# wilsonCernWq/qaray

Hardware: AMD Instinct MI355X
Metric: Msamples/s (1 sample = 1 camera path), Cornell box 1080p@512spp (higher is better)
Workload: dtype f32

## Files before the change

### qaray_amd/csrc/hip/qa_capi.hip

```cpp
#include <hip/hip_runtime.h>

#include <algorithm>
#include <cstddef>
#include <cstring>
#include <new>

#include "qa_ctx.h"

static int EnsurePlanSlab(qa_ctx *c)
{
  const size_t threads = (size_t) c->numCUs * 8 * QA_BLOCK;
  const bool area = c->plan.area, many = !area && c->plan.shadowLights.size() > QA_CS_LIGHT_BATCH;
  float **slab = area ? &c->dAreaSlab : many ? &c->dSurfSlab : nullptr;
  if (slab && !*slab) {
    void *p = nullptr;
    HIP_TRY(hipMalloc(&p, threads * (area ? kAreaLogFloats : 13) * sizeof(float)));
    c->sceneAllocs.push_back(p);
    c->statSceneAllocs++;
    *slab = static_cast<float *>(p);
  }
  c->ds.areaScratch = area ? c->dAreaSlab : nullptr;
  c->ds.csSurf = many ? c->dSurfSlab : nullptr;
  return QA_OK;
}
// ... 351 lines not shown
  if (nbytes) *nbytes = c->hostBlob.size();
  if (!out || capacity < c->hostBlob.size()) return Fail(QA_EINVAL, "output smaller than the scene blob");
  if (int rc = FetchDeviceTexels(c)) return rc;
  memcpy(out, c->hostBlob.data(), c->hostBlob.size());
  return QA_OK;
}

int qa_get_scene_stats(qa_ctx *c, uint64_t out[4])
{
  if (!c || !out) return Fail(QA_EINVAL, "null argument");
  out[0] = c->statMeshBuilds; out[1] = c->statSceneAllocs; out[2] = c->statBytesCopied; out[3] = c->statEdits;
  return QA_OK;
}

int qa_synchronize(qa_ctx *c)
{
  if (int rc = Enter(c)) return rc;
  HIP_TRY(hipStreamSynchronize(c->stream));
  return DrainEvents(c);
}

static int SetStop(qa_ctx *c, int stop)
{
  if (!c) return Fail(QA_EINVAL, "null context");
  __atomic_store_n(c->hStop, stop, __ATOMIC_SEQ_CST);
  return QA_OK;
}
int qa_request_stop(qa_ctx *c) { return SetStop(c, 1); }
int qa_clear_stop(qa_ctx *c) { return SetStop(c, 0); }

int qa_get_counters(qa_ctx *c, qa_counters *out)
{
  if (!c || !out) return Fail(QA_EINVAL, "null argument");
  if (int rc = qa_synchronize(c)) return rc;
  DCounters h;
  HIP_TRY(hipMemcpy(&h, c->dCounters, sizeof(h), hipMemcpyDeviceToHost));
  out->samples = h.samples;
  out->casts_normal = h.casts_normal;
  out->casts_shadow = h.casts_shadow;
  out->bvh_nodes = h.bvh_nodes;
  out->tri_tests = h.tri_tests;
  out->pixels = h.pixels;
#ifdef QA_STAMPS
  {
    const double w = (double) std::max<unsigned long long>(h.stamp[9], 1), k = (double) std::max<unsigned long long>(h.stamp[0], 1);
    fprintf(stderr, "[stamps] waves %llu, iterations/wave %.0f, cycles/wave %.3e | share of wave time: fetch+start %.3f, closest %.3f (mesh walks %.3f), shade %.3f, "
            "direct light %.3f (shadow mesh walks %.3f), sample end %.3f, miss branch %.3f, hit before shading %.3f, spawn %.3f\n", h.stamp[9], h.stamp[8] / w, k / w, h.stamp[1] / k, h.stamp[2] / k, h.stamp[3] / k,
            h.stamp[4] / k, h.stamp[5] / k, h.stamp[6] / k, h.stamp[7] / k, h.stamp[10] / k, h.stamp[11] / k, h.stamp[12] / k);
    if (h.stamp[19] || h.stamp[21])
      fprintf(stderr, "[stamps] waves without a camera ray: mesh walks of their closest-hit sweeps %.3f (the camera rays': %.3f), after the sweep %.3f | last-cast queries %.3f (mesh walks %.3f), %llu lanes asked again (of %llu casts)\n",
              h.stamp[19] / k, (h.stamp[3] - (double) h.stamp[19]) / k, h.stamp[20] / k, h.stamp[21] / k, h.stamp[22] / k, h.stamp[23], (unsigned long long) h.casts_normal);
    if (!c->integ[kCs].fn && h.stamp[16])
      fprintf(stderr, "[stamps] turns of empty tiles: %llu of %llu turns (%.3f), share of wave time %.4f\n", h.stamp[16], h.stamp[8], (double) h.stamp[16] / (double) std::max<unsigned long long>(h.stamp[8], 1), h.stamp[15] / k);
    if (c->integ[kCs].fn && h.stamp[11])
      fprintf(stderr, "[stamps] cooperative walks: %llu rounds, %.1f of 64 lanes hold an item on average (lane occupancy of the walks %.3f); %.3f of the rounds are leaf rounds; 'mesh walks' above = the rounds alone\n", h.stamp[11],
              (double) h.stamp[10] / (double) h.stamp[11], (double) h.stamp[10] / (64.0 * (double) h.stamp[11]), (double) h.stamp[12] / (double) h.stamp[11]);
    if (c->integ[kCs].fn)
      fprintf(stderr, "[stamps] closest-hit sweeps without their rounds %.3f, winners' details %.3f, shadow sweeps without their rounds %.3f; lanes sent to the exact walks: %llu closest, %llu shadow (of %llu + %llu casts)\n",
              (h.stamp[13] - (double) h.stamp[3]) / k, h.stamp[14] / k, (h.stamp[17] - (double) h.stamp[6]) / k, h.stamp[15], h.stamp[16], (unsigned long long) h.casts_normal, (unsigned long long) h.casts_shadow);
  }
#endif
  return QA_OK;
}
int qa_reset_counters(qa_ctx *c)
{
  if (!c) return Fail(QA_EINVAL, "null context");
  if (int rc = qa_synchronize(c)) return rc;
  HIP_TRY(hipMemset(c->dCounters, 0, sizeof(DCounters)));
  if (c->wf.dStats) HIP_TRY(hipMemset(c->wf.dStats, 0, sizeof(WfStats)));
  c->wf.iterations = c->wf.raysClosest = c->wf.raysShadow = c->wf.jobs = c->wf.redo = 0;
  return QA_OK;
}

int qa_get_staged_stats(qa_ctx *c, uint64_t out[QA_STAGED_STATS])
{
  if (!c || !out) return Fail(QA_EINVAL, "null argument");
  if (int rc = qa_synchronize(c)) return rc;
  WfStats st;
  memset(&st, 0, sizeof(st));
  if (c->wf.dStats) HIP_TRY(hipMemcpy(&st, c->wf.dStats, sizeof(st), hipMemcpyDeviceToHost));
  const uint64_t v[QA_STAGED_STATS] = {c->wf.iterations, c->wf.raysClosest, c->wf.raysShadow, c->wf.jobs, c->wf.redo, st.jobs, st.nodeSteps,
                                       st.leafSteps, st.triTests, st.redo, st.suspended, st.laneSlots, st.waveRounds};
  memcpy(out, v, sizeof(v));
  return QA_OK;
}

int qa_set_pipeline(qa_ctx *c, int mode)
{
  if (!c) return Fail(QA_EINVAL, "null context");
  if (mode < QA_PIPE_MEGA || mode > QA_PIPE_AUTO) return Fail(QA_EINVAL, "pipeline mode must be QA_PIPE_MEGA, QA_PIPE_STAGED or QA_PIPE_AUTO");
  c->wf.mode = mode;
  c->wf.modeSet = true;
  if (c->haveScene) SetKernelName(c);
  return QA_OK;
}

const char *qa_get_kernel_name(qa_ctx *c)
{
  if (!c || !c->haveScene) return "";
  return c->launchedName.empty() ? c->kernelName.c_str() : c->launchedName.c_str();
}

int qa_get_kernel_time(qa_ctx *c, double *total_ms, uint64_t *launches)
{
  if (!c || !total_ms || !launches) return Fail(QA_EINVAL, "null argument");
  HIP_TRY(hipSetDevice(c->device));
// ... 54 lines not shown
```

### qaray_amd/csrc/hip/qa_kernel.h

```cpp
#pragma once
#include <hip/hip_runtime.h>

#include <type_traits>

#include "qa_device_math.h"
#include "qa_scene_dev.h"
#include "qa_seed.h"
#include "qa_texture_dev.h"
#include "qa_tilecull.h"
#include "qa_emptytile.h"

namespace qa {

#ifndef QA_MIN_WAVES
#define QA_MIN_WAVES 4
#endif
#define QA_BIAS 0.005f
#define QA_DX 0.01f
#ifdef QA_WAVE_TALLIES
#define QA_TALLY(x) (x) += (unsigned long long) __popcll(__ballot(1))
#else
#define QA_LANE_TALLIES 1
#define QA_TALLY(x) (x)++
#endif
// ... 712 lines not shown
    any |= hit;
  }
  if (any) {
    for (int a = h.node; a >= 0; a = instAt<RES>(sc, a).parent) {
      if (a == 0 && sc.rootIdentity) {
        h.N = normalize(h.N);
        break;
      }
      const qa_instance &in = instAt<RES>(sc, a);
      h.p = mulMV(in.tm, h.p) + ld3(in.pos);
      h.N = normalize(mulTMV(in.itm, h.N));
    }
  }
  return any;
}

template <bool RES, bool STATS>
__device__ __forceinline__ float shadow(const SceneMem<RES> mem, const DScene &sc, const Ray &world, float t_max,
                                        uint32_t *stack, DCounters &cnt)
{
  QA_TALLY(cnt.casts_shadow);
  Hit h;
  h.z = t_max;
  h.node = -1;
  const Ray r0 = rootRay<RES>(sc, world);
  GroupRay grp;
  grp.node = -1;
  grp.ray = r0;
  for (int k = 1; k < sc.num_inst; ++k) {
    const int type = instAt<RES>(sc, k).obj_type;
    if (type == QA_OBJ_NONE) continue;
    const Ray r = localRayInGroup<RES>(sc, k, r0, grp);
    bool hit;
    if (type == QA_OBJ_SPHERE) hit = hitSphere(r, h, k, false);
    else if (type == QA_OBJ_PLANE) hit = hitPlane(r, h, k, false);
    else {
      TriPick pick;
      QA_T(tm0)
      hit = hitMesh<RES, STATS>(mem, meshAt<RES>(sc, instAt<RES>(sc, k).mesh), r, h, k, false, stack, cnt, pick, sc.stackDepth);
      QA_TACC(cnt.sl[6], tm0)
    }
    if (hit) return 0.0f;
  }
  return 1.0f;
}

#ifndef QA_LEAF_SWEEP
#define QA_LEAF_SWEEP 1
#endif
#ifndef QA_LEAF_SWEEP_SORTED
#define QA_LEAF_SWEEP_SORTED 1
#endif

typedef const __attribute__((address_space(4))) uint32_t *QaLeafPtr;
__device__ __forceinline__ uint32_t sweepLeafBoxes(QaLeafPtr rec, uint32_t j0, uint32_t j1, const Ray &ray, f3 pLo, f3 pHi, f3 drcp, bool fastSlab, float limit)
{
  uint32_t mask = 0;
#pragma unroll 4
  for (uint32_t j = j0; j < j1; ++j) {
    QaLeafPtr r = rec + 8 * (size_t) j;
    const f3 bmin = F3(asF(r[0]), asF(r[1]), asF(r[2])), bmax = F3(asF(r[3]), asF(r[4]), asF(r[5]));
    float entry, exit_;
    if (fastSlab) {
#if QA_FMA_SLAB
      boxEntryExitPadFma(pLo, pHi, drcp, bmin, bmax, entry, exit_);
#else
      boxEntryExitPadFast(pLo, pHi, drcp, bmin, bmax, entry, exit_);
#endif
    } else boxEntryExitPad(pLo, pHi, ray.d, drcp, bmin, bmax, entry, exit_);
    mask |= (entry <= limit && entry <= exit_) ? (1u << (j - j0)) : 0u;
  }
  return mask;
}

__device__ __forceinline__ bool sweepLeaves(const uint4 *table, uint32_t numLeaves, const uint4 *ftris, const Ray &ray, f3 drcp, bool fastSlab,
                                            float &hz, uint32_t &best, bool &tie, float pad)
{
  f3 pLo = ray.p + F3(pad, pad, pad), pHi = ray.p - F3(pad, pad, pad);
  if (QA_FMA_SLAB && fastSlab) { pLo = slabRayTerm(pLo, drcp); pHi = slabRayTerm(pHi, drcp); }
  QaLeafPtr rec = (QaLeafPtr) table;
  const uint32_t n0 = numLeaves < 32u ? numLeaves : 32u;
  uint32_t lo = sweepLeafBoxes(rec, 0, n0, ray, pLo, pHi, drcp, fastSlab, hz), hi = 0;
  if (numLeaves > 32u) hi = sweepLeafBoxes(rec, 32, numLeaves, ray, pLo, pHi, drcp, fastSlab, hz);
  typedef const __attribute__((address_space(1))) uint32_t *WordPtr;
  WordPtr words = (WordPtr) table;
  while (lo | hi) {
    uint32_t j;
    if (lo) { j = (uint32_t) __ffs((int) lo) - 1u; lo &= lo - 1u; }
    else { j = 31u + (uint32_t) __ffs((int) hi); hi &= hi - 1u; }
    const uint32_t word = words[8 * (size_t) j + 6];
    const uint32_t count = ((word >> QA_BVH_COUNT_SHIFT) & QA_BVH_COUNT_MASK) + 1;
    const uint32_t first = word & QA_BVH_OFFSET_MASK;
    for (uint32_t i = 0; i < count; ++i) {
      const uint4 *t = ftris + 3 * (size_t) (first + i);
      const uint4 t2 = t[2];
      if (hitTriangleZTie<true>(t[0], t[1], t2, ray, hz, tie)) {
        best = t2.w >> 2;
        return true;
      }
    }
  }
  return false;
}

template <bool RES>
__device__ __forceinline__ bool blocksMesh(const SceneMem<RES> mem, const DMesh &m, const Ray &ray, float limit, uint32_t *stack,
                                           DCounters &cnt, bool &again, const uint4 *leafTable = nullptr)
{
  const f3 drcp = F3(1.f / ray.d.x, 1.f / ray.d.y, 1.f / ray.d.z);
  const bool fastSlab = !__any(qabs(ray.d.x) < 1e-7f || qabs(ray.d.y) < 1e-7f || qabs(ray.d.z) < 1e-7f);
  float meshExit;
  bool gate;
  {
    float entry;
    if (fastSlab) boxEntryExitFast(ray, drcp, ld3(m.bmin), ld3(m.bmax), entry, meshExit);
    else boxEntryExit(ray, drcp, ld3(m.bmin), ld3(m.bmax), entry, meshExit);
    if (entry > meshExit) return false;
    gate = !(entry > limit);
  }
  if (m.num_faces == 0) return false;
  if (!m.useFast) {
    again = true;
    return false;
  }
  const uint4 *nodes = mem.img + m.resNodes, *fnodes = mem.img + m.resFNodes, *ftris = mem.img + m.resFTris;
  const float oMax = qmax(qmax(qabs(ray.p.x), qabs(ray.p.y)), qabs(ray.p.z));
  const float pad = fastWalkPad(m.invH, m.absMax, oMax);
  float hz = limit;
  uint32_t bestF = 0;
  bool tie = false;
  bool hit;
#if QA_LEAF_SWEEP
  const uint32_t numLeaves = __builtin_amdgcn_readfirstlane(m.numLeaves);
  if (leafTable && numLeaves >= 2 && numLeaves <= QA_TILE_LEAF_CAP)
    hit = sweepLeaves(leafTable + __builtin_amdgcn_readfirstlane(m.resLeaves) + (QA_LEAF_SWEEP_SORTED ? 2 * (size_t) numLeaves : 0), numLeaves, ftris, ray,
                      drcp, fastSlab, hz, bestF, tie, pad);
  else
#endif
  hit = walkBVH<true, false, false, QA_BLOCK, QA_FMA_SLAB != 0>(fnodes, ftris, m.frootData, ray, drcp, fastSlab, hz, false, stack, cnt, bestF, tie, pad);
  if (tie) {
    again = true;
    return false;
  }
  if (!hit) {
    if (limit > meshExit) {
      const float theta = ((QA_SLACK_SCALE * 1.8e-5f) * m.invH) * (oMax + m.absMax) + QA_SLACK_SCALE * 2e-5f;
      const float lim = (theta * theta) * dot(ray.d, ray.d);
      bool parallel = m.numNormals == 0;
      const float4 *nrm = reinterpret_cast<const float4 *>(mem.img + m.resNormals);
      for (uint32_t i = 0; i < m.numNormals; ++i) {
        const float4 n = nrm[i];
        const float dn = __builtin_fmaf(ray.d.x, n.x, __builtin_fmaf(ray.d.y, n.y, ray.d.z * n.z));
        parallel = parallel || (dn * dn <= lim);
      }
      if (parallel) {
        uint32_t bestR = 0;
        hz = limit;
        return walkBVH<false, false>(nodes, mem.img + m.resTris, m.rootData, ray, drcp, fastSlab, hz, false, stack, cnt, bestR, tie);
      }
    }
    return false;
  }
  if (!gate || !refReaches(nodes, bestF >> 15, ray, drcp, fastSlab, limit)) {
    again = true;
    return false;
  }
  return true;
}

#ifndef QA_LAST_CAST_ANYHIT
#define QA_LAST_CAST_ANYHIT 1
#endif
template <bool RES>
__device__ __forceinline__ void closestEmitter(const SceneMem<RES> mem, const DScene &sc, const Ray &world, uint32_t *stack,
                                               DCounters &cnt, bool &drawn, int &emitSet)
{
  const Ray r0 = rootRay<RES>(sc, world);
  Hit h;
  h.z = QA_BIGFLOAT;
  h.node = -1;
  for (int k = 1; k < sc.num_inst; ++k) {
    const int type = instAt<RES>(sc, k).obj_type;
    if (type == QA_OBJ_NONE) continue;
    const Ray r = localRay<RES>(sc, k, r0);
    if (type == QA_OBJ_SPHERE) hitSphere(r, h, k, true);
    else if (type == QA_OBJ_PLANE) hitPlane(r, h, k, true);
    else {
      TriPick pick;
      hitMesh<RES, false, true, false>(mem, meshAt<RES>(sc, instAt<RES>(sc, k).mesh), r, h, k, true, stack, cnt, pick, sc.stackDepth);
    }
  }
  drawn = h.node >= 0;
  emitSet = -1;
  for (uint32_t rest = sc.lastCastGlow; rest; rest &= rest - 1) {
    const int k = __ffs((int) rest) - 1;
    if (k == h.node) emitSet = instAt<RES>(sc, k).mtlset;
  }
}

template <bool RES>
__device__ __forceinline__ bool lastCastQuery(const SceneMem<RES> mem, const DScene &sc, const Ray &world, uint32_t *stack,
                                              DCounters &cnt, bool &drawn, int &emitSet)
{
  const Ray r0 = rootRay<RES>(sc, world);
  const uint32_t glow = sc.lastCastGlow;
  Hit h;
  h.z = QA_BIGFLOAT;
  int G = -1, setG = -1;
  for (uint32_t rest = glow; rest; rest &= rest - 1) {
    const int k = __ffs((int) rest) - 1;
    if (k >= sc.num_inst) break;
    const qa_instance &in = instAt<RES>(sc, k);
    const Ray r = localRay<RES>(sc, k, r0);
    const bool hit = in.obj_type == QA_OBJ_SPHERE ? hitSphere(r, h, k, false) : hitPlane(r, h, k, false);
    if (hit) {
      G = k;
      setG = in.mtlset;
    }
  }
  const float tG = h.z;
  const float tGup = __uint_as_float(__float_as_uint(tG) + 1u);
  bool blocked = false, again = false;
  for (int k = 1; k < sc.num_inst; ++k) {
    if ((glow >> k) & 1u) continue;
    const int type = instAt<RES>(sc, k).obj_type;
    if (type == QA_OBJ_NONE) continue;
    const bool open = !blocked && !again;
    if (!__any(open)) break;
    if (open) {
      const float limit = G < 0 ? QA_BIGFLOAT : (k < G ? tGup : tG);
      const Ray r = localRay<RES>(sc, k, r0);
      Hit b;
      b.z = limit;
      if (type == QA_OBJ_SPHERE) blocked = hitSphere(r, b, k, false);
      else if (type == QA_OBJ_PLANE) blocked = hitPlane(r, b, k, false);
      else {
        QA_T(tm0)
        blocked = blocksMesh<RES>(mem, meshAt<RES>(sc, instAt<RES>(sc, k).mesh), r, limit, stack, cnt, again, sc.lastCast == 2u ? sc.resident : nullptr);
        QA_TACC(cnt.sl[22], tm0)
      }
    }
  }
  drawn = blocked || G >= 0;
  emitSet = blocked ? -1 : setG;
  return !again;
}

__device__ __forceinline__ float inverseSquareFalloff(f3 v) { return qmin(1.f, 1.f / dot(v, v)); }

__device__ __forceinline__ float spotAttenuation(const qa_light &l, f3 p)
{
  const f3 d = normalize(p - ld3(l.position));
  const float cosTheta = dot(d, ld3(l.direction));
  if (cosTheta < 0) return 0;
  const float rr = qsqrt(1.f - cosTheta * cosTheta) / cosTheta;
  if (rr > l.outer) return 0;
  return rr < l.inner ? 1.f : qpowf((l.outer - rr) / (l.outer - l.inner), 2.f);
}

template <bool RES, bool STATS>
__device__ __forceinline__ f3 illuminate(const SceneMem<RES> mem, const DScene &sc, const qa_light &l, f3 p,
                                         uint32_t *stack, DCounters &cnt, uint32_t &rng)
{
  const f3 intensity = ld3(l.intensity);
  if (l.type != QA_LIGHT_DIRECT && l.size > 0.01f) {
    int spp = 16, n = 0;
    float inshadow = 0.0f;
    while (n < spp) {
      const f3 dir = (ld3(l.position) + uniformBall(rng, l.size)) - p;
      Ray r;
      r.p = p;
      r.d = normalize(dir);
      inshadow += (shadow<RES, STATS>(mem, sc, r, length(dir), stack, cnt) - inshadow) * inverseSquareFalloff(dir) / (float) (n + 1);
      n++;
      if (inshadow > 0.f && inshadow < 1.f) spp = 64;
    }
    f3 I = intensity * inshadow;
    if (l.type == QA_LIGHT_SPOT) I = I * spotAttenuation(l, p);
    return I;
  }
  if (l.type == QA_LIGHT_DIRECT) {
    Ray r;
    r.p = p;
    r.d = normalize(-ld3(l.direction));
    return intensity * shadow<RES, STATS>(mem, sc, r, QA_BIGFLOAT, stack, cnt);
  }
  const f3 dir = ld3(l.position) - p;
  Ray r;
  r.p = p;
  r.d = normalize(dir);
  f3 I = (intensity * shadow<RES, STATS>(mem, sc, r, length(dir), stack, cnt)) * inverseSquareFalloff(dir);
// ... 429 lines not shown
```

### qaray_amd/csrc/hip/qa_kernel_lastcast_body.h

```cpp
  extern __shared__ uint4 s_dyn[];
  SceneMem<RES> mem;
  mem.img = s_dyn;
  static_assert(RES, "the last-cast query belongs to the resident variant without lights");
  for (uint32_t i = threadIdx.x; i < sc.residentVec4; i += QA_BLOCK) s_dyn[i] = sc.resident[i];
  __syncthreads();
  uint32_t *stack = reinterpret_cast<uint32_t *>(s_dyn + sc.residentVec4) + threadIdx.x;
  float *acc = reinterpret_cast<float *>(stack + (size_t) sc.stackDepth * QA_BLOCK - threadIdx.x) + threadIdx.x;
  const uint4 *mtlTable = s_dyn + sc.resMaterials;
  for (int i = 12; i < QA_LANE_SLOTS_RES; ++i) acc[i * QA_BLOCK] = 0.f;
  constexpr bool TL = true;
  uint32_t *tileList = nullptr;
  if (rp.tile_lists > 0 && !(sc.cam.dof > 0.1f))
    tileList = reinterpret_cast<uint32_t *>(s_dyn + sc.residentVec4) + ((size_t) sc.stackDepth + QA_LANE_SLOTS_RES) * QA_BLOCK +
               __builtin_amdgcn_readfirstlane(threadIdx.x / 64) * QA_TILE_LIST_DWORDS;

  const int rw = rp.x1 - rp.x0, rh = rp.y1 - rp.y0;
  const unsigned tilesX = (unsigned) (rw + 7) / 8;
  const unsigned numTiles = tilesX * (unsigned) rp.own_tile_rows;
  const unsigned total = numTiles * (rp.chunk_spp ? rp.num_chunks : 1u) * 64u;
  const unsigned lane = __lane_id();
  unsigned curTile = 0xFFFFFFFFu, curChunk = 0;
  int chunkEnd = 0x7FFFFFFF;

  DCounters cnt = {};
#ifdef QA_STAMPS
  __shared__ unsigned long long s_stamps[QA_BLOCK / 64][QA_NSTAMPS];
  cnt.sl = s_stamps[threadIdx.x / 64];
  if (__lane_id() < QA_NSTAMPS) cnt.sl[__lane_id()] = 0;
#endif
  QA_T(tKernel)
  TexTables tt;
  tt.blob = sc.blob;
  tt.texels = sc.texels;
  tt.texOff = sc.texOff;
  tt.texmap = sc.texmap;
  tt.tex = sc.tex;
  tt.filter = sc.texFilter;
  RayDiff pathDiff;
  pathDiff.dx = pathDiff.dy = F3(0, 0, 1);

  uint32_t rng = 1;
  bool alive = true, needPixel = true;
#if QA_EMPTY_TILES
#ifdef QA_WAVE_TALLIES
#define QA_TALLY_N(x, n) (x) += (unsigned long long) (n) * (unsigned long long) __popcll(__ballot(1))
#else
#define QA_TALLY_N(x, n) (x) += (unsigned long long) (n)
#endif
#ifdef QA_STAMPS
  bool tileEmpty = false;
#define QA_EMPTY_ASK true
#else
#define QA_EMPTY_ASK (rp.empty_tiles != 0)
#endif
#endif

  for (;;) {
// ... 169 lines not shown
          L = L + T * c;
          QA_TACC(cnt.sl[10], tM)
        } else {
          if (!primary && !h.front && absorbMtl >= 0) {
            const uint4 ab = mtlTable[6 * (size_t) absorbMtl + 5];
            const f3 att = F3(qexpf(-asF(ab.x) * h.z), qexpf(-asF(ab.y) * h.z), qexpf(-asF(ab.z) * h.z));
            T = T * att;
          }
          const qa_instance &in = instAt<RES>(sc, h.node);
          int mi = -1;
          bool white = false;
          if (in.mtlset >= 0) {
            const qa_mtlset ms = sc.mtlset[in.mtlset];
            if (ms.multi) {
              if (h.mtlID >= 0 && h.mtlID < ms.count) mi = ms.first + h.mtlID;
              else white = true;
            } else mi = ms.first;
          }
          if (mi < 0) {
            if (white) L = L + T;
          } else {
            const f3 V = -ray.d;
            const f3 N = h.N;
            const f3 p = h.p;
            QA_TACC(cnt.sl[11], tM)
            QA_T(tD)
            const Surface sf = shadeSurface<false, DScene, false>(mtlTable, sc, tt, mi, N, V, h.front, th, bounce, fromDiffuse, rng);
            QA_TACC(cnt.sl[4], tD)
            L = L + T * sf.emission;
            QA_T(tS)
            if (sf.spawn) {
              ray.p = p;
              ray.d = normalize(sf.nextDir);
              T = T * sf.bxdf;
              absorbMtl = mi;
              bounce -= 1;
              fromDiffuse = sf.nextFromDiffuse;
              go = true;
            }
            QA_TACC(cnt.sl[12], tS)
          }
        }
#ifdef QA_STAMPS
        if (!primary) QA_TACC(cnt.sl[20], tM)
#endif
      }
      if (trip) break;
      primary = false;
      if (sc.lastCast && go) {
        QA_T(tQ)
        bool drawn;
        int emitSet;
#if QA_LAST_CAST_ANYHIT
        go = !lastCastQuery<RES>(mem, sc, ray, stack, cnt, drawn, emitSet);
#else
        closestEmitter<RES>(mem, sc, ray, stack, cnt, drawn, emitSet);
        go = false;
#endif
        if (!go) {
          QA_TALLY(cnt.casts_normal);
          f3 c = ld3(sc.environment);
          if (drawn) {
            (void) rng1(rng);
            c = F3(0, 0, 0);
            if (emitSet >= 0) {
              const uint4 m2 = mtlTable[6 * (size_t) sc.mtlset[emitSet].first + 2];
              c = F3(asF(m2.x), asF(m2.y), asF(m2.z));
            }
          }
          L = L + T * c;
        }
        QA_TACC(cnt.sl[21], tQ)
#ifdef QA_STAMPS
        {
          const unsigned long long asked = __ballot(go);
          if ((int) __lane_id() == __ffsll((long long) __ballot(1)) - 1) cnt.sl[23] += (unsigned long long) __popcll(asked);
        }
#endif
      }
      if (!__any(go)) break;
    }

    QA_T(tE)
#ifdef QA_STAMPS
    if (lane == 0) cnt.sl[8] += 1;
#endif
    if (active) {
      int sidx = __float_as_int(acc[14 * QA_BLOCK]);
      const unsigned qo = __float_as_uint(acc[13 * QA_BLOCK]);
      const f3 pL = L;
      const float inv = (float) (sidx + 1);
      f3 mean = F3(acc[0], acc[QA_BLOCK], acc[2 * QA_BLOCK]);
      f3 cstd = F3(0, 0, 0);
      const f3 dc = (pL - mean) / inv;
      mean = mean + dc;
      acc[0] = mean.x; acc[QA_BLOCK] = mean.y; acc[2 * QA_BLOCK] = mean.z;
      if (rp.spp_min < rp.spp_max) {
        cstd = F3(acc[3 * QA_BLOCK], acc[4 * QA_BLOCK], acc[5 * QA_BLOCK]);
        if (sidx > 0) cstd = cstd + ((dc * dc) * inv - cstd / (float) sidx);
        acc[3 * QA_BLOCK] = cstd.x; acc[4 * QA_BLOCK] = cstd.y; acc[5 * QA_BLOCK] = cstd.z;
      }
      ++sidx;
      acc[14 * QA_BLOCK] = __int_as_float(sidx);
      const bool more = sidx < rp.spp_min ||
                        (sidx < rp.spp_max && (cstd.x > 0.005f || cstd.y > 0.001f || cstd.z > 0.005f));
      if (more) {
        if (rp.chunk_spp && sidx >= chunkEnd) {
// ... 50 lines not shown
```

### qaray_amd/csrc/hip/qa_scene_build.cpp

```cpp
#include "qa_scene_build.h"

#include <algorithm>
#include <cmath>
#include <cstring>
#include <new>

#include "qa_device_math.h"
#include "qa_fastbvh.h"
#include "qa_texel_dev.h"
#include "qa_tilecull.h"
#include "qaray_host.h"

namespace qa {
namespace {

struct Refused { int code; const char *msg; };
[[noreturn]] void Refuse(int code, const char *msg) { throw Refused{code, msg}; }

struct Blob {
  const unsigned char *p;
  size_t n;
  const qa_flat_header *h;
  bool inside(uint64_t off, uint64_t bytes) const { return off <= n && bytes <= n - off; }
  template <class T> const T *at(uint64_t off) const { return QA_BLOB_PTR(T, p, off); }
// ... 498 lines not shown
    if (tx.type == QA_TEX_CHECKER || tx.width <= 0 || tx.height <= 0) continue;
    const size_t n = (size_t) tx.width * (size_t) tx.height;
    if (!b.inside(tx.off_texels, 3 * n)) Refuse(QA_EINVAL, "texture texels outside the blob");
    const unsigned char *px = b.p + tx.off_texels;
    const size_t at = tex4.size();
    tex4.resize(at + 4 * n);
    texelsTabulateHost(px, n, 1, 3 * n, tex4.data() + at);
  }
  if (tex4.size() / 4 > 0xFFFFFFFFull) Refuse(QA_EUNSUPPORTED, "more than 2^32 texels");
  if (tex4.empty()) tex4.assign(4, 0.f);
  out.taps.resize(62);
  for (int i = 1; i < 32; ++i) {
    float x = HaltonF(i, 2), y = HaltonF(i, 3);
    const float r = sqrtf(x) * 0.5f;
    x = r * sinf(y * (float) M_PI * 2);
    y = r * cosf(y * (float) M_PI * 2);
    out.taps[2 * (i - 1)] = x;
    out.taps[2 * (i - 1) + 1] = y;
  }
}

void BuildImage(SceneTables &out)
{
  std::vector<uint4> &image = out.image;
  auto append = [&](const void *p, size_t bytes) {
    const uint32_t off = (uint32_t) image.size();
    const size_t n = (bytes + 15) / 16;
    image.resize(image.size() + n, uint4{0, 0, 0, 0});
    if (bytes) memcpy(image.data() + off, p, bytes);
    return off;
  };
  auto pad64 = [&] { while (image.size() % 4) image.push_back(uint4{0, 0, 0, 0}); };
  for (size_t mi = 0; mi < out.mesh.size(); ++mi) {
    const MeshTables &mt = out.mesh[mi];
    DMesh &dm = out.plan.meshes[mi];
    pad64();
    dm.resNodes = append(mt.nodes.data(), mt.nodes.size() * sizeof(DNode));
    dm.resTris = append(mt.tris.data(), mt.tris.size() * sizeof(DTri));
    dm.resShade = append(mt.shade.data(), mt.shade.size() * sizeof(DTriShade));
    pad64();
    dm.resFNodes = append(mt.fnodes.data(), mt.fnodes.size() * sizeof(DNode));
    dm.resFTris = append(mt.ftris.data(), mt.ftris.size() * sizeof(DTri));
    dm.resFMap = append(mt.fmap.data(), mt.fmap.size() * sizeof(uint32_t));
    dm.resNormals = append(mt.normals.data(), mt.normals.size() * sizeof(float));
    dm.numNormals = (uint32_t) (mt.normals.size() / 4);
  }
  out.ds.resMaterials = append(out.materials.data(), out.materials.size() * sizeof(DMaterial));
  out.imageLdsVec4 = image.size();
  for (size_t mi = 0; mi < out.mesh.size(); ++mi) {
    DMesh &dm = out.plan.meshes[mi];
    dm.numLeaves = dm.useFast ? (uint32_t) out.mesh[mi].leaves.size() : 0u;
    dm.resLeaves = dm.numLeaves ? append(out.mesh[mi].leaves.data(), out.mesh[mi].leaves.size() * sizeof(DNode)) : 0u;
    if (dm.numLeaves) append(out.mesh[mi].sweepLeaves.data(), out.mesh[mi].sweepLeaves.size() * sizeof(DNode));
  }
}

void PlanLastCast(const Blob &b, SceneTables &out);
void PlanScene(const Blob &b, const BuildKnobs &k, uint32_t stackNeedMax, SceneTables &out)
{
  const qa_flat_header *h = b.h;
  DScene &ds = out.ds;
  ScenePlan &plan = out.plan;
  ds.stackNeed = stackNeedMax;
  ds.stackDepth = std::max(stackNeedMax, 8u);
  const size_t stackBytes = ((size_t) ds.stackDepth + QA_LANE_SLOTS) * QA_BLOCK * sizeof(uint32_t);
  const size_t imageBytes = out.imageLdsVec4 * sizeof(uint4);
  if (stackBytes > kMaxLdsPerBlock) Refuse(QA_EUNSUPPORTED, "BVH too deep for the LDS traversal stack");
  const size_t stackBytesRes = ((size_t) ds.stackDepth + QA_LANE_SLOTS_RES) * QA_BLOCK * sizeof(uint32_t);
  plan.resident = imageBytes > 0 && imageBytes + stackBytesRes <= kResidentLdsBudget && h->num_instances <= QA_KARG_INST &&
                  h->num_meshes <= QA_KARG_MESH;
  plan.ldsBytes = plan.resident ? stackBytesRes + imageBytes : stackBytes;
  plan.tileListBytes = 0;
  const size_t listBytes = (QA_BLOCK / 64) * QA_TILE_LIST_DWORDS * sizeof(uint32_t), cuLds = 160 * 1024, unit = 1280;
  auto perCU = [&](size_t bytes) { return cuLds / ((bytes + unit - 1) / unit * unit); };
  bool anyLeaves = false;
  for (const DMesh &dm : plan.meshes) anyLeaves = anyLeaves || dm.numLeaves > 0;
  if (plan.resident && anyLeaves && perCU(plan.ldsBytes + listBytes) == perCU(plan.ldsBytes)) plan.tileListBytes = listBytes;
  if (plan.resident) {
    ds.residentVec4 = (uint32_t) out.imageLdsVec4;
    std::copy(b.at<qa_instance>(h->off_instances), b.at<qa_instance>(h->off_instances) + h->num_instances, ds.instv);
  } else ds.resMaterials = 0;
  ds.csSlots = std::min(std::max(k.csSlots, 64u), 256u);
  ds.csItems = std::max(k.csItems, 128u);
  memcpy(ds.cam.screenA, h->screenA, 12);
  memcpy(ds.cam.screenU, h->screenU, 12);
  memcpy(ds.cam.screenV, h->screenV, 12);
  memcpy(ds.cam.screenX, h->screenX, 12);
  memcpy(ds.cam.screenY, h->screenY, 12);
  memcpy(ds.cam.pos, h->cam_pos, 12);
  ds.cam.dof = h->dof;
  ds.cam.width = (int) h->width;
  ds.cam.height = (int) h->height;
  memcpy(ds.background, h->background.color, 12);
  memcpy(ds.environment, h->environment.color, 12);
  ds.bgTexmap = h->background.texmap;
  ds.envTexmap = h->environment.texmap;
  ds.num_inst = (int) h->num_instances;
  ds.num_lights = (int) h->num_lights;
  ds.num_materials = (int) h->num_materials;
  PlanLastCast(b, out);
}

void PlanLightsAndRoot(const Blob &b, SceneTables &out)
{
  const qa_flat_header *h = b.h;
  ScenePlan &plan = out.plan;
// ... 17 lines not shown
    out.texLayout[i] = TexLayout{textures[i].type, textures[i].width, textures[i].height, 0, textures[i].off_texels};
}

void PlanLastCast(const Blob &b, SceneTables &out)
{
  const qa_flat_header *h = b.h;
  ScenePlan &plan = out.plan;
  plan.lastCastQuery = false;
  plan.lastCastGlow = 0;
  if (h->num_lights != 0 || plan.textured || plan.area || h->num_instances > 32) return;
  const qa_material *mats = b.at<qa_material>(h->off_materials);
  const qa_mtlset *sets = b.at<qa_mtlset>(h->off_mtlsets);
  const qa_instance *inst = b.at<qa_instance>(h->off_instances);
  const qa_mesh *meshes = b.at<qa_mesh>(h->off_meshes);
  auto emits = [&](int32_t mi) { const float *e = mats[mi].emission.color; return !(e[0] == 0.f && e[1] == 0.f && e[2] == 0.f); };
  for (uint32_t i = 0; i < h->num_materials; ++i) {
    const qa_material &m = mats[i];
    for (int k = 0; k < 3; ++k)
      if (m.reflection.color[k] != 0.f || m.refraction.color[k] != 0.f || !(m.absorption[k] == 0.f)) return;
  }
  uint32_t glow = 0;
  for (uint32_t k = 0; k < h->num_instances; ++k) {
    const qa_instance &in = inst[k];
    if (in.obj_type == QA_OBJ_NONE) continue;
    if (k == 0) continue;
    if (in.mtlset < 0 || (uint32_t) in.mtlset >= h->num_mtlsets) return;
    const qa_mtlset &ms = sets[in.mtlset];
    const int32_t count = ms.multi ? ms.count : 1;
    if (ms.first < 0 || count < 1 || (uint64_t) ms.first + (uint64_t) count > h->num_materials) return;
    bool glows = false;
    for (int32_t i = 0; i < count; ++i) glows = glows || emits(ms.first + i);
    if (in.obj_type == QA_OBJ_MESH) {
      if (glows) return;
      if (in.mesh < 0 || (uint32_t) in.mesh >= h->num_meshes) return;
      if (ms.multi) {
        const qa_mesh &m = meshes[in.mesh];
        const qa_face *faces = b.at<qa_face>(m.off_faces);
        for (uint32_t f = 0; f < m.num_faces; ++f)
          if (faces[f].mtl < 0 || faces[f].mtl >= ms.count) return;
      }
    } else {
      if (ms.multi) return;
      if (glows) glow |= 1u << k;
    }
  }
  plan.lastCastQuery = true;
  plan.lastCastGlow = glow;
}

int SyncAuto(const ScenePlan &plan, bool anySpecularLobes) { return (!anySpecularLobes || plan.textured) ? 1 : 0; }

}

float HaltonF(int index, int base)
{
  float r = 0;
  float f = 1.0f / (float) base;
  for (int i = index; i > 0; i /= base) {
    r += f * (i % base);
    f /= (float) base;
  }
  return r;
}

int BuildScene(const unsigned char *blob, size_t nbytes, const BuildKnobs &knobs, SceneTables &out, std::string *err)
{
  out = SceneTables{};
  memset(&out.ds, 0, sizeof(out.ds));
  try {
    const Blob b{blob, nbytes, reinterpret_cast<const qa_flat_header *>(blob)};
    CheckHeader(b);
    const qa_flat_header *h = b.h;
    ScenePlan &plan = out.plan;
    PlanLightsAndRoot(b, out);
    const qa_instance *inst = b.at<qa_instance>(h->off_instances);
    plan.meshInstanced.assign(h->num_meshes, false);
    for (uint32_t k = 0; k < h->num_instances; ++k) if (inst[k].obj_type == QA_OBJ_MESH) plan.meshInstanced[inst[k].mesh] = true;
    plan.textured = h->num_texmaps > 0;
    KeepTexLayout(b, out);
    plan.csFits = true;
    uint32_t stackNeedMax = 1;
    BuildMeshes(b, knobs, out, &stackNeedMax);
    const bool anySpecularLobes = BuildMaterials(b, out);
    BuildImage(out);
    BuildCsTrees(b, out);
    out.csFitsMeshes = plan.csFits;
    BuildCsInstances(b, out);
    plan.syncAuto = SyncAuto(plan, anySpecularLobes);
    if (plan.textured) BuildTextures(b, out);
    PlanScene(b, knobs, stackNeedMax, out);
  } catch (const Refused &r) {
    *err = r.msg;
    return r.code;
  } catch (const std::bad_alloc &) {
    *err = "out of memory";
    return QA_ENOMEM;
  }
  return QA_OK;
}

}

namespace qa {

int RebuildSceneSide(const unsigned char *blob, size_t nbytes, const BuildKnobs &knobs, SceneTables &out, std::string *err)
{
// ... 48 lines not shown
```

### qaray_amd/csrc/hip/qa_scene_build.h

```cpp
#pragma once
#include <hip/hip_runtime.h>

#include <cstdio>
#include <string>
#include <vector>

#include "qa_scene_dev.h"
#include "qa_tilecull.h"
#include "qa_widebvh.h"

namespace qa {

constexpr size_t kMaxLdsPerBlock = 64 * 1024;
constexpr size_t kResidentLdsBudget = 40 * 1024;

struct BuildKnobs {
  bool wide = true;
  unsigned wideLeaf = 3;
  unsigned fastLeaf = 2;
  uint32_t fastMaxFaces = 0xFFFFFFFFu;
  uint32_t csItems = 576, csSlots = 80;
  FILE *report = nullptr;
};

struct MeshTables {
  std::vector<DNode> nodes, fnodes;
  std::vector<DTri> tris, ftris, wtris;
  std::vector<DTriShade> shade;
  std::vector<uint32_t> fmap;
  std::vector<DNode> leaves;
  std::vector<DNode> sweepLeaves;
  std::vector<float> vt;
  std::vector<float> normals;
  WideBvh wide;
};

struct ScenePlan {
  std::vector<DMesh> meshes;
  std::vector<bool> meshInstanced;
  std::vector<int32_t> shadowLights;
  bool textured = false, area = false, resident = false;
  bool csFits = false;
  bool csCullOk = false;
  int syncAuto = 0;
  size_t ldsBytes = 0;
  size_t tileListBytes = 0;
  bool lastCastQuery = false;
  uint32_t lastCastGlow = 0;
};
inline bool MissesTexcoords(const ScenePlan &p, const DMesh &m) { return p.textured && m.num_faces > 0 && !m.hasVT; }

struct TexLayout { int32_t type, width, height, pad; uint64_t off_texels; };

struct SceneTables {
  ScenePlan plan;
  DScene ds{};
  std::vector<MeshTables> mesh;
  std::vector<DWideNode> csNodes;
  std::vector<DTri> csTris;
  std::vector<float> csLeafBox;
  std::vector<CsInst> csInst;
  std::vector<CsCull> csCull;
  std::vector<DMaterial> materials;
  std::vector<int32_t> mtlTex;
  std::vector<float> texels;
  std::vector<uint32_t> texOff;
  std::vector<float> taps;
  std::vector<TexLayout> texLayout;
  std::vector<uint4> image;
  size_t imageLdsVec4 = 0;
  bool csFitsMeshes = false;
  uint32_t meshBuilds = 0;
};

float HaltonF(int index, int base);
int BuildScene(const unsigned char *blob, size_t nbytes, const BuildKnobs &knobs, SceneTables &out, std::string *err);
int RebuildSceneSide(const unsigned char *blob, size_t nbytes, const BuildKnobs &knobs, SceneTables &tables, std::string *err);
void DropMeshSide(SceneTables &tables);

}
```

### qaray_amd/csrc/hip/qa_scene_dev.h

```cpp
#pragma once
#include <stdint.h>

#include "qa_flat_scene.h"
#include "qa_photon.h"

#define QA_BLOCK 256
#define QA_DONE 0xFFFFFFFFu
#define QA_CS_INDEX_MASK 0xFFFFFu
#define QA_CS_LIGHT_BATCH 4
#define QA_CS_EXACT_STACK 64

namespace qa {

struct alignas(32) DNode {
  float box[6];
  uint32_t data;
  uint32_t pad;
};

struct alignas(16) DTri {
  float N[3];
  float A[3];
  float bu, bv, cu, cv;
  float s;
// ... 14 lines not shown
  float specular[3], gloss_spec;
  float emission[3], ior;
  float reflection[3], gloss_refl;
  float refraction[3], gloss_refr;
  float absorption[3];
  uint32_t flags;
};
static_assert(sizeof(DMaterial) == 96, "DMaterial must be 6 x 16 bytes");
#define QA_MTL_SPECULAR_LOBES 1u
#define QA_MTL_HAS_SPECULAR 2u

struct alignas(64) DWideNode {
  float origin[3];
  float scale[3];
  uint32_t lo[3];
  uint32_t hi[3];
  uint32_t child[4];
};
static_assert(sizeof(DWideNode) == 64, "DWideNode must be 4 x 16 bytes");

struct DMesh {
  float bmin[3], bmax[3];
  const DNode *nodes;
  const DTri *tris;
  const DTriShade *shade;
  uint32_t num_faces, num_nodes;
  uint32_t rootData;
  uint32_t stackNeed;
  uint32_t resNodes, resTris, resShade;
  uint32_t hasVT;
  const float *vt;
  const DNode *fnodes;
  const DTri *ftris;
  const uint32_t *fmap;
  uint32_t frootData;
  uint32_t useFast;
  float invH;
  float absMax;
  uint32_t numNormals;
  uint32_t resNormals;
  uint32_t resFNodes, resFTris, resFMap;
  uint32_t gateIsRoot;
  const DWideNode *wnodes;
  const DTri *wtris;
  uint32_t wrootWord;
  uint32_t useWide;
  uint32_t wnodeCount;
  uint32_t wideStack;
  float nearPad;
  float cancelDist;
  uint32_t csRootWord;
  uint32_t resLeaves;
  uint32_t numLeaves;
  uint32_t leafPad;
};

#ifndef QA_SLACK_SCALE
#define QA_SLACK_SCALE 1.0f
#endif

struct alignas(64) CsInst {
  float itmA[9], posA[3];
  float itmB[9], posB[3];
  float tmA[9], tmB[9];
  int32_t type, depth;
  uint32_t useWide, csRootWord, num_faces, mesh;
  float bmin[3], bmax[3];
  float nearPad, absMax, cancelDist;
  float wmin[3], wmax[3];
  int32_t parent;
};
static_assert(sizeof(CsInst) == 256, "CsInst must be 64 dwords");

struct alignas(32) CsCull {
  float lo[3], pad0;
  float hi[3], pad1;
};
static_assert(sizeof(CsCull) == 32, "CsCull must be 8 dwords");

#define QA_LANE_SLOTS 6
#define QA_LANE_SLOTS_RES 15
#define QA_KARG_INST 12
#define QA_KARG_MESH 4

struct DCamera {
  float screenA[3], screenU[3], screenV[3], screenX[3], screenY[3], pos[3];
  float dof;
  int32_t width, height;
};

struct DScene {
  const unsigned char *blob;
  const qa_instance *inst;
  const qa_mtlset *mtlset;
  const DMaterial *mtl;
  const qa_light *light;
  const DMesh *mesh;
  const float *halton;
  const uint4 *resident;
  const qa_texmap *texmap;
  const qa_texture *tex;
  const float4 *texels;
  const uint32_t *texOff;
  const float *texFilter;
  float *areaScratch;
  const int32_t *mtlTex;
  DCamera cam;
// ... 78 lines not shown
```

Baseline: 29620.

## Encode leaf triangle pairs as LDS bytes and test both triangles per sweep turn

At scene build, each sorted sweep leaf holding at most two triangles with a small offset is packed into one byte, and these bytes are appended after the leaf table. The last-cast kernel copies the bytes into shared memory, and the leaf sweep then tests both triangles of a leaf in one loop turn, with no per-leaf global word load and no inner count loop. The aim is less divergent inner looping and fewer memory reads in the shadow any-hit sweep. In exchange, a single-triangle leaf costs a redundant second test, and meshes that do not meet the packing limits fall back to the full BVH walk. It also adds stamp counters that split the sweep into its box and triangle phases.

```diff
diff --git a/qaray_amd/csrc/hip/qa_capi.hip b/qaray_amd/csrc/hip/qa_capi.hip
--- a/qaray_amd/csrc/hip/qa_capi.hip
+++ b/qaray_amd/csrc/hip/qa_capi.hip
@@ -427,6 +427,9 @@
               h.stamp[19] / k, (h.stamp[3] - (double) h.stamp[19]) / k, h.stamp[20] / k, h.stamp[21] / k, h.stamp[22] / k, h.stamp[23], (unsigned long long) h.casts_normal);
     if (!c->integ[kCs].fn && h.stamp[16])
       fprintf(stderr, "[stamps] turns of empty tiles: %llu of %llu turns (%.3f), share of wave time %.4f\n", h.stamp[16], h.stamp[8], (double) h.stamp[16] / (double) std::max<unsigned long long>(h.stamp[8], 1), h.stamp[15] / k);
+    if (!c->integ[kCs].fn && h.stamp[17])
+      fprintf(stderr, "[stamps] leaf sweep: box phase %.4f, triangle phase %.4f of wave time | triangle phase: %.1f turns per wave, %.2f of 64 lanes in a turn, %.1f cycles per turn\n", h.stamp[13] / k, h.stamp[14] / k,
+              h.stamp[17] / w, (double) h.stamp[18] / (double) h.stamp[17], (double) h.stamp[14] / (double) h.stamp[17]);
     if (c->integ[kCs].fn && h.stamp[11])
       fprintf(stderr, "[stamps] cooperative walks: %llu rounds, %.1f of 64 lanes hold an item on average (lane occupancy of the walks %.3f); %.3f of the rounds are leaf rounds; 'mesh walks' above = the rounds alone\n", h.stamp[11],
               (double) h.stamp[10] / (double) h.stamp[11], (double) h.stamp[10] / (64.0 * (double) h.stamp[11]), (double) h.stamp[12] / (double) h.stamp[11]);
diff --git a/qaray_amd/csrc/hip/qa_kernel.h b/qaray_amd/csrc/hip/qa_kernel.h
--- a/qaray_amd/csrc/hip/qa_kernel.h
+++ b/qaray_amd/csrc/hip/qa_kernel.h
@@ -788,6 +788,19 @@
 #define QA_LEAF_SWEEP_SORTED 1
 #endif
 
+#ifndef QA_LEAF_PAIR
+#define QA_LEAF_PAIR 1
+#endif
+#if defined(QA_STAMPS)
+#define QA_SWEEP_TURN(cnt)                                                                          \
+  {                                                                                                 \
+    const unsigned long long in_ = __ballot(1);                                                     \
+    if ((int) __lane_id() == __ffsll((long long) in_) - 1) { cnt.sl[17] += 1; cnt.sl[18] += (unsigned long long) __popcll(in_); } \
+  }
+#else
+#define QA_SWEEP_TURN(cnt)
+#endif
+
 typedef const __attribute__((address_space(4))) uint32_t *QaLeafPtr;
 __device__ __forceinline__ uint32_t sweepLeafBoxes(QaLeafPtr rec, uint32_t j0, uint32_t j1, const Ray &ray, f3 pLo, f3 pHi, f3 drcp, bool fastSlab, float limit)
 {
@@ -810,14 +823,41 @@
 }
 
 __device__ __forceinline__ bool sweepLeaves(const uint4 *table, uint32_t numLeaves, const uint4 *ftris, const Ray &ray, f3 drcp, bool fastSlab,
-                                            float &hz, uint32_t &best, bool &tie, float pad)
+                                            float &hz, uint32_t &best, bool &tie, float pad, DCounters &cnt, const uint8_t *pairs = nullptr)
 {
   f3 pLo = ray.p + F3(pad, pad, pad), pHi = ray.p - F3(pad, pad, pad);
   if (QA_FMA_SLAB && fastSlab) { pLo = slabRayTerm(pLo, drcp); pHi = slabRayTerm(pHi, drcp); }
   QaLeafPtr rec = (QaLeafPtr) table;
   const uint32_t n0 = numLeaves < 32u ? numLeaves : 32u;
+  QA_T(tBox)
   uint32_t lo = sweepLeafBoxes(rec, 0, n0, ray, pLo, pHi, drcp, fastSlab, hz), hi = 0;
   if (numLeaves > 32u) hi = sweepLeafBoxes(rec, 32, numLeaves, ray, pLo, pHi, drcp, fastSlab, hz);
+  QA_TACC(cnt.sl[13], tBox)
+  QA_T(tTri)
+#if QA_LEAF_PAIR
+  bool found = false;
+  while ((lo | hi) && !found) {
+    QA_SWEEP_TURN(cnt)
+    uint32_t j;
+    if (lo) { j = (uint32_t) __ffs((int) lo) - 1u; lo &= lo - 1u; }
+    else { j = 31u + (uint32_t) __ffs((int) hi); hi &= hi - 1u; }
+    const uint32_t byte = pairs[j];
+    const uint4 *t = ftris + 3 * (size_t) (byte & 127u), *u = t + 3 * (size_t) (byte >> 7);
+    const uint4 t2 = t[2], u2 = u[2];
+    float h1 = hz, h2 = hz;
+    bool tie1 = false, tie2 = false;
+    const bool ok1 = hitTriangleZTie<true>(t[0], t[1], t2, ray, h1, tie1);
+    const bool ok2 = hitTriangleZTie<true>(u[0], u[1], u2, ray, h2, tie2);
+    tie = tie || tie1 || (!ok1 && tie2);
+    found = ok1 || ok2;
+    if (found) {
+      best = (ok1 ? t2.w : u2.w) >> 2;
+      hz = ok1 ? h1 : h2;
+    }
+  }
+  QA_TACC(cnt.sl[14], tTri)
+  return found;
+#else
   typedef const __attribute__((address_space(1))) uint32_t *WordPtr;
   WordPtr words = (WordPtr) table;
   while (lo | hi) {
@@ -828,20 +868,24 @@
     const uint32_t count = ((word >> QA_BVH_COUNT_SHIFT) & QA_BVH_COUNT_MASK) + 1;
     const uint32_t first = word & QA_BVH_OFFSET_MASK;
     for (uint32_t i = 0; i < count; ++i) {
+      QA_SWEEP_TURN(cnt)
       const uint4 *t = ftris + 3 * (size_t) (first + i);
       const uint4 t2 = t[2];
       if (hitTriangleZTie<true>(t[0], t[1], t2, ray, hz, tie)) {
         best = t2.w >> 2;
+        QA_TACC(cnt.sl[14], tTri)
         return true;
       }
     }
   }
+  QA_TACC(cnt.sl[14], tTri)
   return false;
+#endif
 }
 
 template <bool RES>
 __device__ __forceinline__ bool blocksMesh(const SceneMem<RES> mem, const DMesh &m, const Ray &ray, float limit, uint32_t *stack,
-                                           DCounters &cnt, bool &again, const uint4 *leafTable = nullptr)
+                                           DCounters &cnt, bool &again, const uint4 *leafTable = nullptr, const uint8_t *leafPairs = nullptr)
 {
   const f3 drcp = F3(1.f / ray.d.x, 1.f / ray.d.y, 1.f / ray.d.z);
   const bool fastSlab = !__any(qabs(ray.d.x) < 1e-7f || qabs(ray.d.y) < 1e-7f || qabs(ray.d.z) < 1e-7f);
@@ -868,9 +912,13 @@
   bool hit;
 #if QA_LEAF_SWEEP
   const uint32_t numLeaves = __builtin_amdgcn_readfirstlane(m.numLeaves);
+#if QA_LEAF_PAIR
+  if (leafTable && numLeaves >= 2 && numLeaves <= QA_TILE_LEAF_CAP && m.leafPairs && leafPairs)
+#else
   if (leafTable && numLeaves >= 2 && numLeaves <= QA_TILE_LEAF_CAP)
+#endif
     hit = sweepLeaves(leafTable + __builtin_amdgcn_readfirstlane(m.resLeaves) + (QA_LEAF_SWEEP_SORTED ? 2 * (size_t) numLeaves : 0), numLeaves, ftris, ray,
-                      drcp, fastSlab, hz, bestF, tie, pad);
+                      drcp, fastSlab, hz, bestF, tie, pad, cnt, leafPairs);
   else
 #endif
   hit = walkBVH<true, false, false, QA_BLOCK, QA_FMA_SLAB != 0>(fnodes, ftris, m.frootData, ray, drcp, fastSlab, hz, false, stack, cnt, bestF, tie, pad);
@@ -936,7 +984,7 @@
 
 template <bool RES>
 __device__ __forceinline__ bool lastCastQuery(const SceneMem<RES> mem, const DScene &sc, const Ray &world, uint32_t *stack,
-                                              DCounters &cnt, bool &drawn, int &emitSet)
+                                              DCounters &cnt, bool &drawn, int &emitSet, const uint8_t *leafPairs = nullptr)
 {
   const Ray r0 = rootRay<RES>(sc, world);
   const uint32_t glow = sc.lastCastGlow;
@@ -972,7 +1020,13 @@
       else if (type == QA_OBJ_PLANE) blocked = hitPlane(r, b, k, false);
       else {
         QA_T(tm0)
+#if QA_LEAF_PAIR
+        const int mi = instAt<RES>(sc, k).mesh;
+        blocked = blocksMesh<RES>(mem, meshAt<RES>(sc, mi), r, limit, stack, cnt, again, sc.lastCast == 2u ? sc.resident : nullptr,
+                                  leafPairs ? leafPairs + QA_TILE_LEAF_CAP * (size_t) mi : nullptr);
+#else
         blocked = blocksMesh<RES>(mem, meshAt<RES>(sc, instAt<RES>(sc, k).mesh), r, limit, stack, cnt, again, sc.lastCast == 2u ? sc.resident : nullptr);
+#endif
         QA_TACC(cnt.sl[22], tm0)
       }
     }
diff --git a/qaray_amd/csrc/hip/qa_kernel_lastcast_body.h b/qaray_amd/csrc/hip/qa_kernel_lastcast_body.h
--- a/qaray_amd/csrc/hip/qa_kernel_lastcast_body.h
+++ b/qaray_amd/csrc/hip/qa_kernel_lastcast_body.h
@@ -3,6 +3,15 @@
   mem.img = s_dyn;
   static_assert(RES, "the last-cast query belongs to the resident variant without lights");
   for (uint32_t i = threadIdx.x; i < sc.residentVec4; i += QA_BLOCK) s_dyn[i] = sc.resident[i];
+#if QA_LEAF_PAIR
+  static_assert(QA_KARG_MESH * QA_TILE_LEAF_CAP <= 6 * QA_BLOCK * sizeof(uint32_t), "the leaf-pair bytes live in columns 6 to 11");
+  uint32_t *const leafPairWords = reinterpret_cast<uint32_t *>(s_dyn + sc.residentVec4) + ((size_t) sc.stackDepth + 6) * QA_BLOCK;
+  for (int mi = 0; mi < QA_KARG_MESH; ++mi) {
+    const DMesh &pm = sc.meshv[mi];
+    if (pm.leafPairs && threadIdx.x < QA_TILE_LEAF_CAP / 4)
+      leafPairWords[mi * (QA_TILE_LEAF_CAP / 4) + threadIdx.x] = reinterpret_cast<const uint32_t *>(sc.resident + pm.resLeaves + 4 * (size_t) pm.numLeaves)[threadIdx.x];
+  }
+#endif
   __syncthreads();
   uint32_t *stack = reinterpret_cast<uint32_t *>(s_dyn + sc.residentVec4) + threadIdx.x;
   float *acc = reinterpret_cast<float *>(stack + (size_t) sc.stackDepth * QA_BLOCK - threadIdx.x) + threadIdx.x;
@@ -278,7 +287,11 @@
         bool drawn;
         int emitSet;
 #if QA_LAST_CAST_ANYHIT
+#if QA_LEAF_PAIR
+        go = !lastCastQuery<RES>(mem, sc, ray, stack, cnt, drawn, emitSet, reinterpret_cast<const uint8_t *>(s_dyn + sc.residentVec4) + ((size_t) sc.stackDepth + 6) * QA_BLOCK * sizeof(uint32_t));
+#else
         go = !lastCastQuery<RES>(mem, sc, ray, stack, cnt, drawn, emitSet);
+#endif
 #else
         closestEmitter<RES>(mem, sc, ray, stack, cnt, drawn, emitSet);
         go = false;
diff --git a/qaray_amd/csrc/hip/qa_scene_build.cpp b/qaray_amd/csrc/hip/qa_scene_build.cpp
--- a/qaray_amd/csrc/hip/qa_scene_build.cpp
+++ b/qaray_amd/csrc/hip/qa_scene_build.cpp
@@ -574,6 +574,9 @@
     dm.numLeaves = dm.useFast ? (uint32_t) out.mesh[mi].leaves.size() : 0u;
     dm.resLeaves = dm.numLeaves ? append(out.mesh[mi].leaves.data(), out.mesh[mi].leaves.size() * sizeof(DNode)) : 0u;
     if (dm.numLeaves) append(out.mesh[mi].sweepLeaves.data(), out.mesh[mi].sweepLeaves.size() * sizeof(DNode));
+    unsigned char pairs[QA_TILE_LEAF_CAP];
+    dm.leafPairs = dm.numLeaves && LeafPairBytes(out.mesh[mi].sweepLeaves, pairs) ? 1u : 0u;
+    if (dm.numLeaves) append(pairs, sizeof(pairs));
   }
 }
 
@@ -697,6 +700,22 @@
 
 }
 
+bool LeafPairBytes(const std::vector<DNode> &sorted, unsigned char bytes[QA_TILE_LEAF_CAP])
+{
+  memset(bytes, 0, QA_TILE_LEAF_CAP);
+  if (sorted.empty() || sorted.size() > QA_TILE_LEAF_CAP) return false;
+  for (size_t j = 0; j < sorted.size(); ++j) {
+    const uint32_t word = sorted[j].data;
+    const uint32_t count = ((word >> QA_BVH_COUNT_SHIFT) & QA_BVH_COUNT_MASK) + 1, first = word & QA_BVH_OFFSET_MASK;
+    if (count > 2 || first > 127) {
+      memset(bytes, 0, QA_TILE_LEAF_CAP);
+      return false;
+    }
+    bytes[j] = (unsigned char) (first | (count - 1) << 7);
+  }
+  return true;
+}
+
 float HaltonF(int index, int base)
 {
   float r = 0;
diff --git a/qaray_amd/csrc/hip/qa_scene_build.h b/qaray_amd/csrc/hip/qa_scene_build.h
--- a/qaray_amd/csrc/hip/qa_scene_build.h
+++ b/qaray_amd/csrc/hip/qa_scene_build.h
@@ -73,6 +73,7 @@
   uint32_t meshBuilds = 0;
 };
 
+bool LeafPairBytes(const std::vector<DNode> &sorted, unsigned char bytes[QA_TILE_LEAF_CAP]);
 float HaltonF(int index, int base);
 int BuildScene(const unsigned char *blob, size_t nbytes, const BuildKnobs &knobs, SceneTables &out, std::string *err);
 int RebuildSceneSide(const unsigned char *blob, size_t nbytes, const BuildKnobs &knobs, SceneTables &tables, std::string *err);
diff --git a/qaray_amd/csrc/hip/qa_scene_dev.h b/qaray_amd/csrc/hip/qa_scene_dev.h
--- a/qaray_amd/csrc/hip/qa_scene_dev.h
+++ b/qaray_amd/csrc/hip/qa_scene_dev.h
@@ -90,7 +90,7 @@
   uint32_t csRootWord;
   uint32_t resLeaves;
   uint32_t numLeaves;
-  uint32_t leafPad;
+  uint32_t leafPairs;
 };
 
 #ifndef QA_SLACK_SCALE
```

After: 31130, median of 6. +5.1%, better.
